# anuragranj/cc

Measured on AMD Instinct MI355X. Metric: train images/sec (832x256, 5-frame sample, 6-scale CC step), higher is better.
Workload: dtype f32; 1 GPU; full CC: DispResNet6+PoseNetB6+MaskNet6+Back2Future, all losses; per_gpu_batch=4, global_batch=4, height=256, width=832, scales=6, frames=5, parallelism=dp1, hipgraph=True, trained_nets=all, rccl_ranks=1, dead_occlusion_decoders_elided=False, net_streams=2, pipeline=per_network, grad_chunks=False, deterministic=True

## Files before the change

### cc_amd/csrc/conv_wgrad.hip

```cpp
#include <stdio.h>
#include <stddef.h>
#include <string.h>
#include "cc_common.h"
#include "conv_internal.h"
#include "cc_tools.h"
#include "../../include/ccengine.h"

namespace {

typedef float f32x16 __attribute__((ext_vector_type(16)));

using ccint::BK;
using ccint::BN;
using ccint::MAXGRP;
using ccint::pick_bm;

struct WG {
    const float* a;
    const float* x;
    float* out;
    const float* ga[MAXGRP]; const float* gxp[MAXGRP]; float* gout[MAXGRP];
    int nsplit;
    int B, M, AH, AW; long a_bs;
    int Cin, IH, IW; long x_bs;
    int Rt, St, dy0, dx0, dstep, si;
    long o_sm, o_sc; int o_ri, o_sj;
    int direct, accum;
    int pix_per_split;
};

template <int BM>
__device__ __forceinline__ void wgrad_body(const WG& g, const int bx_, const int by_, const int bz_) {
    const int grp = bz_ / g.nsplit, zsplit = bz_ - grp * g.nsplit;
    const float* __restrict__ a_ = g.ga[grp];
    const float* __restrict__ x_ = g.gxp[grp];
    float* __restrict__ out_ = g.gout[grp];
    constexpr int WM = (BM >= 64) ? BM / 2 : 32;
    constexpr int WN = (BM >= 64) ? 64 : 32;
    constexpr int TM = WM / 32, TN = WN / 32;
    constexpr int AP = BM + 4, BP = BN + 4;
    constexpr int AQ = BM / 16;
    __shared__ float As[2][BK * AP];
    __shared__ float Bs[2][BK * BP];

    const int tid = threadIdx.x, lane = tid & 63;
    const int wid = __builtin_amdgcn_readfirstlane(tid >> 6);
    const int wm = (BM >= 64) ? (wid >> 1) : 0;
    const int wn = (BM >= 64) ? (wid & 1) : wid;
    const int m0 = by_ * BM;
    const int n0 = bx_ * BN;
    const int RS = g.Rt * g.St;
    const int Ntot = g.Cin * RS;
    const int HWa = g.AH * g.AW;
    const long Ptot = (long)g.B * HWa;
    const long pbeg = (long)zsplit * g.pix_per_split;
    long pend = pbeg + g.pix_per_split;
    if (pend > Ptot) pend = Ptot;
    const int x_cs = g.IH * g.IW;

    const int pp = tid & 15, rgp = tid >> 4;
    int xoff[8], tdy[8], tdx[8];
#pragma unroll
    for (int q = 0; q < 8; q++) {
        const int jn = n0 + rgp + 16 * q;
        if (jn < Ntot) {
            const int c = jn / RS, rem = jn - c * RS;
            const int i = rem / g.St, j = rem - i * g.St;
            tdy[q] = g.dy0 + i * g.dstep;
            tdx[q] = g.dx0 + j * g.dstep;
            xoff[q] = c * x_cs + tdy[q] * g.IW + tdx[q];
        } else {
            tdy[q] = -(1 << 28);
            tdx[q] = 0;
            xoff[q] = 0;
        }
    }
    float ra[AQ], rb[8];
    unsigned okA = 0, okB = 0;
    auto load_chunk = [&](long pbase) {
        okA = 0;
        okB = 0;
        const long p = pbase + pp;
        const bool pv = p < pend;
        const long ps = pv ? p : 0;
        const int n = (int)(ps / HWa);
        const int t = (int)(ps - (long)n * HWa);
        const int ty = t / g.AW, tx = t - ty * g.AW;
        const long abase = (long)n * g.a_bs + ty * g.AW + tx;
#pragma unroll
        for (int q = 0; q < AQ; q++) {
            const int m = m0 + rgp + 16 * q;
            const bool ok = pv && (m < g.M);
            ra[q] = a_[ok ? abase + (long)m * HWa : 0];
            okA |= (ok ? 1u : 0u) << q;
        }
        const int iy0 = g.si * ty, ix0 = g.si * tx;
        const long xb = (long)n * g.x_bs + (long)iy0 * g.IW + ix0;
#pragma unroll
        for (int q = 0; q < 8; q++) {
            const int iy = iy0 + tdy[q], ix = ix0 + tdx[q];
            const bool ok = pv && ((unsigned)iy < (unsigned)g.IH) && ((unsigned)ix < (unsigned)g.IW);
            rb[q] = x_[ok ? xb + xoff[q] : 0];
            okB |= (ok ? 1u : 0u) << q;
        }
    };
    auto store_chunk = [&](int buf) {
#pragma unroll
        for (int q = 0; q < AQ; q++) As[buf][pp * AP + rgp + 16 * q] = ((okA >> q) & 1u) ? ra[q] : 0.f;
#pragma unroll
        for (int q = 0; q < 8; q++) Bs[buf][pp * BP + rgp + 16 * q] = ((okB >> q) & 1u) ? rb[q] : 0.f;
    };

    f32x16 acc[TM][TN];
#pragma unroll
    for (int a = 0; a < TM; a++)
#pragma unroll
        for (int b = 0; b < TN; b++)
#pragma unroll
            for (int r = 0; r < 16; r++) acc[a][b][r] = 0.f;

    const int l31 = lane & 31, lk = lane >> 5;
    const long nchunks = (pend > pbeg) ? (pend - pbeg + BK - 1) / BK : 0;
    if (nchunks > 0) {
        load_chunk(pbeg);
        store_chunk(0);
    }
    __syncthreads();
    for (long ch = 0; ch < nchunks; ch++) {
        const int buf = (int)(ch & 1);
        if (ch + 1 < nchunks) load_chunk(pbeg + (ch + 1) * BK);
        {
            float af[BK / 2][TM], bf[BK / 2][TN];
#pragma unroll
            for (int ks = 0; ks < BK / 2; ks++) {
#pragma unroll
                for (int a = 0; a < TM; a++) af[ks][a] = As[buf][(2 * ks + lk) * AP + wm * WM + a * 32 + l31];
#pragma unroll
                for (int b = 0; b < TN; b++) bf[ks][b] = Bs[buf][(2 * ks + lk) * BP + wn * WN + b * 32 + l31];
            }
#pragma unroll
            for (int ks = 0; ks < BK / 2; ks++)
#pragma unroll
                for (int a = 0; a < TM; a++)
#pragma unroll
                    for (int b = 0; b < TN; b++)
                        acc[a][b] = __builtin_amdgcn_mfma_f32_32x32x2f32(af[ks][a], bf[ks][b], acc[a][b], 0, 0, 0);
        }
        if (ch + 1 < nchunks) store_chunk(buf ^ 1);
        __syncthreads();
    }
#pragma unroll
    for (int b = 0; b < TN; b++) {
        const int jn = n0 + wn * WN + b * 32 + l31;
        if (jn >= Ntot) continue;
        long obase;
        if (g.direct) {
            const int c = jn / RS, rem = jn - c * RS;
            const int i = rem / g.St, j = rem - i * g.St;
            obase = (long)c * g.o_sc + i * g.o_ri + j * g.o_sj;
        } else {
            obase = (long)zsplit * g.M * Ntot + jn;
        }
#pragma unroll
        for (int a = 0; a < TM; a++)
#pragma unroll
            for (int r = 0; r < 16; r++) {
                const int m = m0 + wm * WM + a * 32 + (r & 3) + 8 * (r >> 2) + 4 * lk;
                if (m < g.M) {
                    float* o = out_ + obase + (g.direct ? (long)m * g.o_sm : (long)m * Ntot);
                    *o = (g.direct && g.accum) ? (*o + acc[a][b][r]) : acc[a][b][r];
                }
            }
    }
}

template <int BM>
__global__ __launch_bounds__(256) void k_wgrad(WG g) {
    if constexpr (CC_XCD_MASK & 4) {
        const int gx = (int)gridDim.x, gy = (int)gridDim.y;
        const int b = cc_xcd_order((int)blockIdx.x + gx * ((int)blockIdx.y + gy * (int)blockIdx.z), gx * gy * (int)gridDim.z);
        const int r = b / gx;
        wgrad_body<BM>(g, b - r * gx, r % gy, r / gy);
    } else {
        wgrad_body<BM>(g, (int)blockIdx.x, (int)blockIdx.y, (int)blockIdx.z);
    }
}

constexpr int MAXWCLS = 12;
struct WGM { WG c[MAXWCLS]; int n; int bx_end[MAXWCLS]; int gx[MAXWCLS], gy[MAXWCLS]; };
template <int BM>
__global__ __launch_bounds__(256) void k_wgrad_multi(WGM a) {
    int k = 0, first = 0, end = a.bx_end[0];
#pragma unroll
    for (int q = 0; q < MAXWCLS - 1; q++)
        if (q + 1 < a.n && (int)blockIdx.x >= a.bx_end[q]) { k = q + 1; first = a.bx_end[q]; end = a.bx_end[q + 1]; }
#if defined(__HIP_DEVICE_COMPILE__) && !defined(CC_HIPEMU)
    const WG& g = *(reinterpret_cast<const WG*>((const char*)__builtin_amdgcn_kernarg_segment_ptr() + offsetof(WGM, c)) + k);
#else
    const WG& g = a.c[k];
#endif
    const int b = (CC_XCD_MASK & 4) ? cc_xcd_order((int)blockIdx.x - first, end - first) : (int)blockIdx.x - first;
    const int gx = a.gx[k], gy = a.gy[k];
    const int bx = b % gx, r = b / gx;
    wgrad_body<BM>(g, bx, r % gy, r / gy);
}

constexpr int W3_PC = 41;

struct W3 {
    const float* a; const float* x; const float* zeros; float* ws;
    const float* ga[MAXGRP]; const float* gxp[MAXGRP]; float* gws[MAXGRP];
    int B, M, AH, AW; long a_bs;
    int Cin; long x_bs;
    int tiles_x, tiles_y, ntiles, tiles_per_split, nsplit, Cpad, dbg;
};

template <int MT, int CT>
__global__ __launch_bounds__(256, 2) void k_wgrad3x3(W3 g) {
    const float* __restrict__ a_ = g.ga[blockIdx.y];
    const float* __restrict__ x_ = g.gxp[blockIdx.y];
    float* __restrict__ ws_ = g.gws[blockIdx.y];
    constexpr int BM = 32 * MT, BC = 32 * CT;
    constexpr int A_SLOTS = BM * 16;
    constexpr int P_SLOTS = ((BC * W3_PC + 63) / 64) * 64;
    HIP_DYNAMIC_SHARED(float, smem)
    float4* As = reinterpret_cast<float4*>(smem);
    float4* Ps = reinterpret_cast<float4*>(smem) + A_SLOTS;

    const int tid = threadIdx.x, lane = tid & 63;
    const int wid = __builtin_amdgcn_readfirstlane(tid >> 6);
    const int l31 = lane & 31, lk = lane >> 5;
    const int ctiles = g.Cpad / BC;
    const int ctile = blockIdx.x % ctiles, mtile = blockIdx.x / ctiles;
    const int m0 = mtile * BM, c0 = ctile * BC;
    const int HW = g.AH * g.AW;
    const int pt_beg = blockIdx.z * g.tiles_per_split;
    int pt_end = pt_beg + g.tiles_per_split;
    if (pt_end > g.ntiles) pt_end = g.ntiles;

    int g_row[3], g_mt[3], g_ct[3];
    f32x16 acc[3][3];
#pragma unroll
    for (int k = 0; k < 3; k++) {
        const int gi = wid + 4 * k;
        g_row[k] = gi % 3;
        const int tl = gi / 3;
        g_mt[k] = tl % MT;
        g_ct[k] = tl / MT;
#pragma unroll
        for (int j = 0; j < 3; j++)
#pragma unroll
            for (int r = 0; r < 16; r++) acc[k][j][r] = 0.f;
    }

    auto load_tile = [&](int pt) {
        const int tile_x = pt % g.tiles_x;
        const int r2 = pt / g.tiles_x;
        const int tile_y = r2 % g.tiles_y;
        const int n = r2 / g.tiles_y;
        const int ty0 = tile_y * 2, tx0 = tile_x * 32;
        for (int s0 = wid * 64; s0 < A_SLOTS; s0 += 256) {
            const int sl = s0 + lane;
            const int mm = sl >> 4, sc = sl & 15;
            const int pc = sc ^ (mm & 15);
            const int ty = ty0 + (pc >> 3), tx = tx0 + 4 * (pc & 7);
            const int m = m0 + mm;
            const bool ok = (m < g.M) && (ty < g.AH) && (tx < g.AW);
            const float* src = ok ? a_ + (long)n * g.a_bs + (long)m * HW + (long)ty * g.AW + tx : g.zeros;
            __builtin_amdgcn_global_load_lds(CC_GLOBAL_PTR(src), CC_LDS_PTR(As + s0), 16, 0, 0);
        }
        for (int s0 = wid * 64; s0 < P_SLOTS; s0 += 256) {
            const int sl = s0 + lane;
            const int cc = sl / W3_PC, r = sl - cc * W3_PC;
            const int py = r / 10, ch = r - py * 10;
            const int iy = ty0 - 1 + py, ix = tx0 - 4 + 4 * ch;
            const int c = c0 + cc;
            const bool ok = (cc < BC) && (r < 40) && (c < g.Cin) && ((unsigned)iy < (unsigned)g.AH) && ((unsigned)ix < (unsigned)g.AW);
            const float* src = ok ? x_ + (long)n * g.x_bs + (long)c * HW + (long)iy * g.AW + ix : g.zeros;
            __builtin_amdgcn_global_load_lds(CC_GLOBAL_PTR(src), CC_LDS_PTR(Ps + s0), 16, 0, 0);
        }
    };

    for (int pt = pt_beg; pt < pt_end; pt++) {
        if (pt > pt_beg) __syncthreads();
        if (!(g.dbg & 1) || pt == pt_beg) load_tile(pt);
        CC_WAIT_VMCNT0();
        __syncthreads();
        if (g.dbg & 2) continue;
#pragma unroll
        for (int row = 0; row < 2; row++) {
#pragma unroll 2
            for (int pq = 0; pq < 4; pq++) {
#pragma unroll
                for (int k = 0; k < 3; k++) {
                    const int mrow = g_mt[k] * 32 + l31;
                    float4 av = As[mrow * 16 + ((row * 8 + pq + 4 * lk) ^ (mrow & 15))];
                    const float4* Pr = Ps + (g_ct[k] * 32 + l31) * W3_PC + (row + g_row[k]) * 10 + 4 * lk + pq;
                    float4 w0 = Pr[0], w1 = Pr[1], w2 = Pr[2];
                    CC_KEEP4(av); CC_KEEP4(w0); CC_KEEP4(w1); CC_KEEP4(w2);
                    const float a[4] = {av.x, av.y, av.z, av.w};
                    const float w[12] = {w0.x, w0.y, w0.z, w0.w, w1.x, w1.y, w1.z, w1.w, w2.x, w2.y, w2.z, w2.w};
#pragma unroll
                    for (int e = 0; e < 4; e++)
#pragma unroll
                        for (int j = 0; j < 3; j++)
                            acc[k][j] = __builtin_amdgcn_mfma_f32_32x32x2f32(a[e], w[3 + j + e], acc[k][j], 0, 0, 0);
                }
            }
        }
    }
#pragma unroll
    for (int k = 0; k < 3; k++) {
#pragma unroll
        for (int j = 0; j < 3; j++) {
            float* o = ws_ + (((long)blockIdx.z * 9 + (g_row[k] * 3 + j)) * g.M) * g.Cpad + c0 + g_ct[k] * 32 + l31;
#pragma unroll
            for (int r = 0; r < 16; r++) {
                const int m = m0 + g_mt[k] * 32 + (r & 3) + 8 * (r >> 2) + 4 * lk;
                if (m < g.M) o[(long)m * g.Cpad] = acc[k][j][r];
            }
        }
    }
}

__global__ void k_zero64(float* p) { p[threadIdx.x] = 0.f; }

struct WgGeom { int B, M, AH, AW, Cin, IH, IW, R, S, si, pad; };

struct W3Plan { bool ok; int mt, nbuf, tiles_x, tiles_y, ntiles, nsplit, tps, Cp32; size_t smem, ws_floats; };

inline W3Plan plan_w3(int B, int M, int AH, int AW, int Cin, int R, int S, int si, int pad, int IH, int IW, int G = 1) {
    W3Plan p = {};
    p.ok = (R == 3 && S == 3 && si == 1 && pad == 1 && IH == AH && IW == AW && (AW % 4) == 0 && AW >= 16 && Cin >= 32 &&
            M >= cctools::env_int("CC_W3_MINM", 64) &&
            !cctools::env_flag("CC_NO_WGRAD3X3"));
    if (!p.ok) return p;
    p.mt = (M > 64) ? 4 : ((M > 32 && Cin > 32) ? 2 : ((Cin > 64) ? 1 : 2));
    p.nbuf = 1;
    const int BM = 32 * p.mt, BC = 32 * (4 / p.mt);
    p.Cp32 = ((Cin + BC - 1) / BC) * BC;
    p.tiles_x = (AW + 31) / 32;
    p.tiles_y = (AH + 1) / 2;
    p.ntiles = B * p.tiles_x * p.tiles_y;
    const long base = (long)((M + BM - 1) / BM) * (p.Cp32 / BC) * (G > 1 ? G : 1);
    long nsplit = (cctools::env_int("CC_W3_SPLIT", 512) + base - 1) / base;
    const long mt_ = cctools::env_int("CC_W3_MINTILES", 3);
    const long cap = (p.ntiles + mt_ - 1) / mt_;
    if (nsplit > cap) nsplit = cap;
    if (nsplit > p.ntiles) nsplit = p.ntiles;
    if (nsplit < 1) nsplit = 1;
    p.tps = (int)((p.ntiles + nsplit - 1) / nsplit);
    p.nsplit = (p.ntiles + p.tps - 1) / p.tps;
    p.smem = (size_t)(BM * 16 + ((BC * W3_PC + 63) / 64) * 64) * 16;
    p.ws_floats = 64 + (size_t)p.nsplit * 9 * M * p.Cp32;
    return p;
}

struct WinoPadPlan { bool ok; int Wp; ccint::WinoWgradPlan wp; size_t pad_floats; };
inline WinoPadPlan wino_pad_plan(int B, int M, int AH, int AW, int Cin, int G) {
    WinoPadPlan p = {};
    if ((AW % 4) == 0 || AH < 2 || cctools::env_flag("CC_NO_WINO_WGRAD_PAD")) return p;
    if (M < cctools::env_int("CC_WWP_MINM", 96) || Cin < cctools::env_int("CC_WWP_MINC", 96)) return p;
    p.Wp = (AW + 3) & ~3;
    p.wp = ccint::wino_wgrad_plan(B, M, AH, p.Wp, Cin, G, cctools::env_int("CC_WWP_MINQ", 64));
    p.ok = p.wp.ok != 0;
    p.pad_floats = ((size_t)B * (Cin + M) * AH * p.Wp + 3) & ~(size_t)3;
    return p;
}

inline long generic_nsplit(long tiles, long P, bool parked) {
    const long target = parked ? cctools::env_int("CC_WGRAD_PARK_TARGET", 256) : cctools::env_int("CC_WGRAD_SPLIT_TARGET", 512);
    long nsplit = (target + tiles - 1) / tiles;
    const long mr = parked ? cctools::env_int("CC_WGRAD_PARK_MINRANGE", 64) : cctools::env_int("CC_WGRAD_MINRANGE", 32);
    const long maxsplit = (P + mr - 1) / mr;
    if (nsplit > maxsplit) nsplit = maxsplit;
    return nsplit < 1 ? 1 : nsplit;
}

enum WgPath { WG_WINO, WG_WINO_PAD, WG_HEAD, WG_THIN, WG_W3, WG_GENERIC };
struct WgCand {
    WgPath path;
    size_t ws_floats;
    char name[64];
    ccint::WinoWgradPlan wino; int Wp;
    ccint::HeadWgradPlan head;
    W3Plan w3;
};
constexpr int WG_MAXCAND = 5;

static int wgrad_candidates(const WgGeom& g, int G, bool sizing, WgCand* out) {
    int n = 0;
    auto add = [&](WgPath path, size_t ws_floats) -> WgCand& {
        out[n] = WgCand{};
        out[n].path = path;
        out[n].ws_floats = ws_floats;
        return out[n++];
    };
    const int pad = sizing ? 1 : g.pad, IH = sizing ? g.AH : g.IH, IW = sizing ? g.AW : g.IW;
    if (g.R == 3 && g.S == 3 && g.si == 1 && pad == 1 && IH == g.AH && IW == g.AW) {
        const ccint::WinoWgradPlan wp = ccint::wino_wgrad_plan(g.B, g.M, g.AH, g.AW, g.Cin, G);
        if (wp.ok) {
            WgCand& c = add(WG_WINO, wp.ws_floats);
            c.wino = wp;
            snprintf(c.name, sizeof c.name, "k_wino_wgrad");
        }
        const WinoPadPlan pp = wino_pad_plan(g.B, g.M, g.AH, g.AW, g.Cin, G);
        if (pp.ok) {
            WgCand& c = add(WG_WINO_PAD, pp.wp.ws_floats + pp.pad_floats);
            c.wino = pp.wp;
            c.Wp = pp.Wp;
            snprintf(c.name, sizeof c.name, "k_wino_wgrad");
        }
        const ccint::HeadWgradPlan hp = g.M <= 2 ? ccint::head_wgrad_plan(g.B, g.M, g.AH, g.AW, g.Cin) : ccint::HeadWgradPlan{};
        if (hp.ok) {
            WgCand& c = add(WG_HEAD, hp.ws_floats);
            c.head = hp;
            snprintf(c.name, sizeof c.name, "k_wgrad_thinm<%d>", g.M);
        }
    }
    {
        char nm[64] = "";
        if (!sizing) ccint::wgrad_thin_name(g.B, g.M, g.AH, g.AW, g.Cin, g.IH, g.IW, g.R, g.S, g.si, g.pad, nm, sizeof nm);
        const size_t wf = ccint::wgrad_thin_ws_floats(g.B, g.M, g.AH, g.AW, g.Cin, g.R, g.S, g.si);
        if (wf && (sizing || nm[0])) memcpy(add(WG_THIN, wf).name, nm, sizeof nm);
    }
    const W3Plan q = plan_w3(g.B, g.M, g.AH, g.AW, g.Cin, g.R, g.S, g.si, pad, IH, IW, G);
    if (q.ok) {
        WgCand& c = add(WG_W3, q.ws_floats);
        c.w3 = q;
        snprintf(c.name, sizeof c.name, "k_wgrad3x3<%d, %d>", q.mt, 4 / q.mt);
    } else {
        const long Ntot = (long)g.Cin * g.R * g.S;
        const int bm = pick_bm(g.M);
        const long nsplit = generic_nsplit(((Ntot + BN - 1) / BN) * ((g.M + bm - 1) / bm), (long)g.B * g.AH * g.AW, false);
        WgCand& c = add(WG_GENERIC, nsplit <= 1 ? 4 : (size_t)nsplit * g.M * Ntot);
        snprintf(c.name, sizeof c.name, "k_wgrad<%d>", bm);
    }
    return n;
}

struct WgradParked { WG g; int bm; dim3 grid; double gflop; };
struct WgradCollector { WgradParked* p; int cap, n; ccint::WinoWgradParked* wino; };

static void launch_wgrad_parked(const WgradCollector& c, hipStream_t s) {
    for (int bm = 128; bm >= 32; bm /= 2) {
        int i = 0;
        while (i < c.n) {
            WGM m = {};
            long blk = 0;
            double gf = 0;
            for (; i < c.n && m.n < MAXWCLS; i++) {
                if (c.p[i].bm != bm) continue;
                const dim3& gr = c.p[i].grid;
                const long nb = (long)gr.x * gr.y * gr.z;
                if (m.n && blk + nb >= (1l << 31)) break;
                m.c[m.n] = c.p[i].g;
                m.gx[m.n] = (int)gr.x; m.gy[m.n] = (int)gr.y;
                blk += nb;
                m.bx_end[m.n] = (int)blk;
                gf += c.p[i].gflop;
                m.n++;
            }
            if (!m.n) break;
            char nm[64];
            snprintf(nm, sizeof nm, "k_wgrad_multi<%d>%s", bm, "");
            cctiming::Scope tsc(nm, gf, s);
            if (bm == 128) hipLaunchKernelGGL(HIP_KERNEL_NAME(k_wgrad_multi<128>), dim3((unsigned)blk), dim3(256), 0, s, m);
            else if (bm == 64) hipLaunchKernelGGL(HIP_KERNEL_NAME(k_wgrad_multi<64>), dim3((unsigned)blk), dim3(256), 0, s, m);
            else hipLaunchKernelGGL(HIP_KERNEL_NAME(k_wgrad_multi<32>), dim3((unsigned)blk), dim3(256), 0, s, m);
        }
    }
}

struct WgCall {
    int G; const long *a, *x, *gw;
    float* ws; size_t stride_f;
    WgGeom g; long a_bs, x_bs, o_sm, o_sc; int accumulate;
    hipStream_t s; ccint::RedSink* sink; const float* zeros64; WgradCollector* park;
    float* area(int k) const { return ws + k * stride_f; }
};
constexpr int WG_DECLINED = 1;

static int emit_slab_reduce(const WgCall& c, float* const* slabs, int nsplit, int Cp) {
    long rd[MAXGRP][ccint::RD_LONGS];
    for (int k = 0; k < c.G; k++) {
        const long d[ccint::RD_LONGS] = {1, (long)slabs[k], (long)c.gw[k], nsplit, c.accumulate, c.o_sm, c.o_sc, 9, c.g.M, c.g.Cin, Cp};
        memcpy(rd[k], d, sizeof d);
    }
    return ccint::wgrad_reduce_emit(c.sink, &rd[0][0], c.G, c.s);
}

static int emit_tile_reduce(const WgCall& c, long nsplit) {
    const WgGeom& g = c.g;
    long rd[MAXGRP][ccint::RD_LONGS];
    for (int k = 0; k < c.G; k++) {
        const long d[ccint::RD_LONGS] = {0, (long)c.area(k), (long)c.gw[k], nsplit, c.accumulate, c.o_sm, c.o_sc, g.M,
                                         (long)g.Cin * g.R * g.S, g.R * g.S, g.S, g.S, 1};
        memcpy(rd[k], d, sizeof d);
    }
    return ccint::wgrad_reduce_emit(c.sink, &rd[0][0], c.G, c.s);
}

static int run_wino(const WgCall& c, const WgCand& cd) {
    const WgGeom& g = c.g;
    const bool padded = cd.path == WG_WINO_PAD;
    const int W = padded ? cd.Wp : g.AW;
    ccint::WinoWgradParked* wpark = c.park ? c.park->wino : nullptr;
    const bool parks = wpark && wpark->n + c.G <= ccint::WINO_WGRAD_PARK_CAP;
    const ccint::WinoWgradPlan wp = parks ? ccint::wino_wgrad_plan_parked(cd.wino, g.M) : cd.wino;
    const size_t slabs = (cd.wino.ws_floats + 3) & ~(size_t)3;
    const float *ap[MAXGRP], *xp[MAXGRP];
    float* wsp[MAXGRP];
    ccint::PadJob jobs[2 * MAXGRP];
    for (int k = 0; k < c.G; k++) {
        ap[k] = (const float*)c.a[k]; xp[k] = (const float*)c.x[k]; wsp[k] = c.area(k) + 64;
        if (padded) {
            float* xpad = c.area(k) + slabs;
            float* apad = xpad + (size_t)g.B * g.Cin * g.AH * W;
            jobs[2 * k] = ccint::PadJob{xp[k], xpad, c.x_bs, g.Cin * g.AH};
            jobs[2 * k + 1] = ccint::PadJob{ap[k], apad, c.a_bs, g.M * g.AH};
            xp[k] = xpad; ap[k] = apad;
        }
    }
    char nm[128];
    int nl = snprintf(nm, sizeof nm, "%s", cd.name);
    if (cctools::env_flag("CC_TIMING_DETAIL")) {
        nl += snprintf(nm + nl, sizeof nm - nl, " G%d B%d M%d C%d %dx%d", c.G, g.B, g.M, g.Cin, g.AH, g.AW);
        if (padded) nl += snprintf(nm + nl, sizeof nm - nl, "(pad %d)", W);
        snprintf(nm + nl, sizeof nm - nl, " k%d wg%d", wp.nsplit, wp.nmb * wp.ncb * c.G * wp.nsplit);
    }
    bool ok;
    {
        cctiming::Scope tsc(nm, 2e-9 * 16.0 * c.G * g.B * ((g.AH + 1) / 2) * ((W + 1) / 2) * (double)g.M * g.Cin, c.s, !parks);
        if (padded) ccint::pad_rows_launch(jobs, 2 * c.G, g.B, g.AW, W, c.s);
        ok = ccint::wino_wgrad_launch(wp, ap, xp, wsp, c.G, g.B, g.M, g.AH, W, padded ? (long)g.M * g.AH * W : c.a_bs, g.Cin,
                                      padded ? (long)g.Cin * g.AH * W : c.x_bs, c.s, wpark);
    }
    return ok ? emit_slab_reduce(c, wsp, wp.nsplit, wp.Cp) : WG_DECLINED;
}

static int run_head(const WgCall& c, const WgCand& cd) {
    const WgGeom& g = c.g;
    const ccint::HeadWgradPlan& hp = cd.head;
    char nm[128];
    const int nl = snprintf(nm, sizeof nm, "%s", cd.name);
    if (cctools::env_flag("CC_TIMING_DETAIL"))
        snprintf(nm + nl, sizeof nm - nl, " G%d B%d M%d C%d %dx%d r3 s1 k%d", c.G, g.B, g.M, g.Cin, g.AH, g.AW, hp.nblk);
    bool ok = true;
    {
        cctiming::Scope tsc(nm, 2e-9 * c.G * g.B * g.AH * g.AW * (double)g.M * g.Cin * 9, c.s);
        for (int k = 0; k < c.G && ok; k++)
            ok = ccint::head_wgrad_launch(hp, (const float*)c.a[k], (const float*)c.x[k], c.area(k), g.B, g.M, g.AH, g.AW, c.a_bs, g.Cin,
                                          c.x_bs, c.s);
    }
    if (!ok) return WG_DECLINED;
    if (cctools::env_flag("CC_HEAD_TRACE"))
        fprintf(stderr, "head wgrad: G%d B%d M%d C%d %dx%d R%d nblk %d\n", c.G, g.B, g.M, g.Cin, g.AH, g.AW, hp.R, hp.nblk);
    return emit_tile_reduce(c, hp.nblk);
}

static int run_thin(const WgCall& c, const WgCand& cd) {
    const WgGeom& g = c.g;
    char nm[128];
    const int nl = snprintf(nm, sizeof nm, "%s", cd.name);
    if (cctools::env_flag("CC_TIMING_DETAIL"))
        snprintf(nm + nl, sizeof nm - nl, " G%d B%d M%d C%d %dx%d r%d s%d", c.G, g.B, g.M, g.Cin, g.AH, g.AW, g.R, g.si);
    cctiming::Scope tsc(nm, 2e-9 * c.G * g.B * g.AH * g.AW * (double)g.M * g.Cin * g.R * g.S, c.s, !ccint::wgrad_thin_parking());
    bool thin = true;
    for (int k = 0; k < c.G && thin; k++)
        thin = ccint::wgrad_thin_launch((const float*)c.a[k], (const float*)c.x[k], (float*)c.gw[k], c.area(k), g.B, g.M, g.AH, g.AW,
                                        c.a_bs, g.Cin, g.IH, g.IW, c.x_bs, g.R, g.S, g.si, g.pad, c.o_sm, c.o_sc, c.accumulate, c.s,
                                        c.sink);
    return thin ? CC_OK : WG_DECLINED;
}

static int run_w3(const WgCall& c, const WgCand& cd) {
    const WgGeom& g = c.g;
    const W3Plan& q = cd.w3;
    W3 w = {};
    w.zeros = c.zeros64 ? c.zeros64 : c.ws;
    for (int k = 0; k < c.G; k++) { w.ga[k] = (const float*)c.a[k]; w.gxp[k] = (const float*)c.x[k]; w.gws[k] = c.area(k) + 64; }
    w.B = g.B; w.M = g.M; w.AH = g.AH; w.AW = g.AW; w.a_bs = c.a_bs; w.Cin = g.Cin; w.x_bs = c.x_bs;
    w.tiles_x = q.tiles_x; w.tiles_y = q.tiles_y; w.ntiles = q.ntiles; w.tiles_per_split = q.tps; w.nsplit = q.nsplit;
    w.Cpad = q.Cp32;
    if (!c.zeros64) hipLaunchKernelGGL(k_zero64, dim3(1), dim3(64), 0, c.s, c.ws);
    const int BM = 32 * q.mt, BC = 32 * (4 / q.mt);
    dim3 grid((unsigned)(((g.M + BM - 1) / BM) * (q.Cp32 / BC)), (unsigned)c.G, (unsigned)q.nsplit);
    w.dbg = cctools::env_int("CC_W3_DBG", 0);
    {
        char nm[128];
        const int nl = snprintf(nm, sizeof nm, "%s", cd.name);
        if (cctools::env_flag("CC_TIMING_DETAIL"))
            snprintf(nm + nl, sizeof nm - nl, " G%d B%d M%d C%d %dx%d k%d wg%d", c.G, g.B, g.M, g.Cin, g.AH, g.AW, q.nsplit,
                     (int)(grid.x * grid.y * grid.z));
        cctiming::Scope tsc(nm, 2e-9 * c.G * g.B * g.AH * g.AW * (double)g.M * g.Cin * 9, c.s);
        if (q.mt == 4) hipLaunchKernelGGL(HIP_KERNEL_NAME(k_wgrad3x3<4, 1>), grid, dim3(256), q.smem, c.s, w);
        else if (q.mt == 2) hipLaunchKernelGGL(HIP_KERNEL_NAME(k_wgrad3x3<2, 2>), grid, dim3(256), q.smem, c.s, w);
        else hipLaunchKernelGGL(HIP_KERNEL_NAME(k_wgrad3x3<1, 4>), grid, dim3(256), q.smem, c.s, w);
    }
    return emit_slab_reduce(c, w.gws, q.nsplit, q.Cp32);
}

static int run_generic(const WgCall& c, const WgCand& cd) {
    const WgGeom& g = c.g;
    const long Ntot = (long)g.Cin * g.R * g.S;
    const long P = (long)g.B * g.AH * g.AW;
    const int bm = pick_bm(g.M);
    const bool parked = c.park && c.park->n < c.park->cap;
    long nsplit = generic_nsplit(((Ntot + BN - 1) / BN) * ((g.M + bm - 1) / bm) * c.G, P, parked);
    long pps = (P + nsplit - 1) / nsplit;
    pps = ((pps + BK - 1) / BK) * BK;
    nsplit = (P + pps - 1) / pps;
    WG w = {};
    w.B = g.B; w.M = g.M; w.AH = g.AH; w.AW = g.AW; w.a_bs = c.a_bs;
    w.Cin = g.Cin; w.IH = g.IH; w.IW = g.IW; w.x_bs = c.x_bs;
    w.Rt = g.R; w.St = g.S; w.dy0 = -g.pad; w.dx0 = -g.pad; w.dstep = 1; w.si = g.si;
    w.o_sm = c.o_sm; w.o_sc = c.o_sc; w.o_ri = g.S; w.o_sj = 1;
    w.direct = (nsplit == 1);
    w.accum = c.accumulate;
    w.nsplit = (int)nsplit;
    for (int k = 0; k < c.G; k++) {
        w.ga[k] = (const float*)c.a[k]; w.gxp[k] = (const float*)c.x[k];
        w.gout[k] = w.direct ? (float*)c.gw[k] : c.area(k);
    }
    w.pix_per_split = (int)pps;
    dim3 grid((unsigned)((Ntot + BN - 1) / BN), (unsigned)((g.M + bm - 1) / bm), (unsigned)(nsplit * c.G));
    const double gflop = 2e-9 * c.G * g.B * g.AH * g.AW * (double)g.M * g.Cin * g.R * g.S;
    if (parked) {
        c.park->p[c.park->n++] = WgradParked{w, bm, grid, gflop};
    } else {
        char nm[128];
        const int nl = snprintf(nm, sizeof nm, "%s", cd.name);
        if (cctools::env_flag("CC_TIMING_DETAIL"))
            snprintf(nm + nl, sizeof nm - nl, " G%d B%d M%d C%d %dx%d r%d s%d k%ld wg%d", c.G, g.B, g.M, g.Cin, g.AH, g.AW, g.R, g.si,
                     (long)nsplit, (int)(grid.x * grid.y * grid.z));
        cctiming::Scope tsc(nm, gflop, c.s);
        if (bm == 128) hipLaunchKernelGGL(HIP_KERNEL_NAME(k_wgrad<128>), grid, dim3(256), 0, c.s, w);
        else if (bm == 64) hipLaunchKernelGGL(HIP_KERNEL_NAME(k_wgrad<64>), grid, dim3(256), 0, c.s, w);
        else hipLaunchKernelGGL(HIP_KERNEL_NAME(k_wgrad<32>), grid, dim3(256), 0, c.s, w);
    }
    return w.direct ? CC_OK : emit_tile_reduce(c, nsplit);
}

}

extern "C" {

size_t cc_conv2d_wgrad_ws_bytes(int B, int M, int AH, int AW, int Cin, int R, int S, int si) {
    const WgGeom g = {B, M, AH, AW, Cin, 0, 0, R, S, si, 0};
    WgCand c[WG_MAXCAND];
    size_t floats = 0;
    for (int G = 1; G <= MAXGRP; G++) {
        const int n = wgrad_candidates(g, G, true, c);
        for (int i = 0; i < n; i++)
            if (c[i].ws_floats > floats) floats = c[i].ws_floats;
    }
    return (floats * sizeof(float) + 15) & ~(size_t)15;
}

static int wgrad_group_impl(int G, const long* a, const long* x, const long* gw, float* ws, int B, int M, int AH, int AW, long a_bs,
                            int Cin, int IH, int IW, long x_bs, int R, int S, int si, int pad, long o_sm, long o_sc, int accumulate,
                            void* stream, ccint::RedSink* sink, const float* zeros64 = nullptr, WgradCollector* park = nullptr) {
    if (G <= 0 || G > MAXGRP || B <= 0 || M <= 0 || Cin <= 0) return CC_ERR_ARG;
    const WgCall c = {G, a, x, gw, ws, cc_conv2d_wgrad_ws_bytes(B, M, AH, AW, Cin, R, S, si) / sizeof(float),
                      WgGeom{B, M, AH, AW, Cin, IH, IW, R, S, si, pad}, a_bs, x_bs, o_sm, o_sc, accumulate,
                      (hipStream_t)stream, sink, zeros64, park};
    WgCand cand[WG_MAXCAND];
    const int n = wgrad_candidates(c.g, G, false, cand);
    for (int i = 0; i < n; i++) {
        const WgCand& cd = cand[i];
        const int r = cd.path == WG_WINO || cd.path == WG_WINO_PAD ? run_wino(c, cd)
                      : cd.path == WG_HEAD ? run_head(c, cd)
                      : cd.path == WG_THIN ? run_thin(c, cd)
                      : cd.path == WG_W3   ? run_w3(c, cd)
                                           : run_generic(c, cd);
        if (r == WG_DECLINED) continue;
        if (r != CC_OK) return CC_ERR_ARG;
        CC_CHECK_LAUNCH();
        return CC_OK;
    }
    return CC_ERR_ARG;
}

int cc_conv2d_wgrad_group(int G, const long* a, const long* x, const long* gw, float* ws, int B, int M, int AH, int AW, long a_bs,
                          int Cin, int IH, int IW, long x_bs, int R, int S, int si, int pad, long o_sm, long o_sc, int accumulate,
                          void* stream) {
    return wgrad_group_impl(G, a, x, gw, ws, B, M, AH, AW, a_bs, Cin, IH, IW, x_bs, R, S, si, pad, o_sm, o_sc, accumulate, stream,
                            nullptr);
}

int cc_conv2d_wgrad_group_defer(int G, const long* a, const long* x, const long* gw, float* ws, int B, int M, int AH, int AW,
                                long a_bs, int Cin, int IH, int IW, long x_bs, int R, int S, int si, int pad, long o_sm, long o_sc,
                                int accumulate, const float* zeros64_or_null, long* red_host, int red_cap, int* nred_host,
                                void* stream) {
    if (!red_host || !nred_host || red_cap < G) return CC_ERR_ARG;
    ccint::RedSink sink = {red_host, red_cap, 0};
    const int r = wgrad_group_impl(G, a, x, gw, ws, B, M, AH, AW, a_bs, Cin, IH, IW, x_bs, R, S, si, pad, o_sm, o_sc, accumulate,
                                   stream, &sink, zeros64_or_null);
    *nred_host = sink.n;
    return r;
}

int cc_conv2d_wgrad_list(int n, const long* desc_host, const float* zeros64_or_null, long* red_host, int red_cap, int* nred_host,
                         void* stream) {
    if (n <= 0 || !desc_host || !red_host || !nred_host) return CC_ERR_ARG;
    hipStream_t s = (hipStream_t)stream;
    constexpr int CAP = 64;
    static thread_local WgradParked parked[CAP];
    static thread_local ccint::WinoWgradParked wino_parked;
    wino_parked.n = 0;
    WgradCollector col = {parked, CAP, 0, cctools::env_flag("CC_NO_WINO_WGRAD_LIST") ? nullptr : &wino_parked};
    ccint::RedSink sink = {red_host, red_cap, 0};
    struct ThinPark {
        hipStream_t s; bool was;
        explicit ThinPark(hipStream_t st) : s(st), was(ccint::wgrad_thin_park(true)) {}
        ~ThinPark() {
            const double gf = ccint::wgrad_thin_parked_gflop();
            if (gf > 0) {
                cctiming::Scope tsc("k_wgrad_thin_multi", gf, s);
                ccint::wgrad_thin_flush(s);
            }
            ccint::wgrad_thin_park(was);
        }
    } thin_park(s);
    for (int i = 0; i < n; i++) {
        const long* d = desc_host + 32l * i;
        const int G = (int)d[0];
        auto bail = [&](int code) {
            launch_wgrad_parked(col, s);
            if (wino_parked.n > 0) ccint::wino_wgrad_launch_parked(&wino_parked, s);
            *nred_host = sink.n;
            return code;
        };
        if (G <= 0 || G > MAXGRP || sink.n + G > red_cap) return bail(CC_ERR_ARG);
        const int before = col.n;
        const int r = wgrad_group_impl(G, d + 1, d + 5, d + 9, (float*)d[13], (int)d[14], (int)d[15], (int)d[16], (int)d[17], d[18],
                                       (int)d[19], (int)d[20], (int)d[21], d[22], (int)d[23], (int)d[24], (int)d[25], (int)d[26], d[27],
                                       d[28], (int)d[29], stream, &sink, zeros64_or_null, &col);
        if (r != CC_OK) return bail(r);
        if (col.n > before && col.p[before].g.direct) {
            bool dup = false;
            for (int j = 0; j < before && !dup; j++)
                if (col.p[j].g.direct)
                    for (int u = 0; u < MAXGRP && !dup; u++)
                        for (int v = 0; v < MAXGRP; v++)
                            if (col.p[j].g.gout[u] && col.p[j].g.gout[u] == col.p[before].g.gout[v]) { dup = true; break; }
            if (dup) {
                const WgradParked keep = col.p[before];
                col.n = before;
                launch_wgrad_parked(col, s);
                col.p[0] = keep;
                col.n = 1;
            }
        }
    }
    launch_wgrad_parked(col, s);
    if (wino_parked.n > 0) {
        double gf = 0;
        for (int i = 0; i < wino_parked.n; i++) gf += wino_parked.d[i].gflop;
        cctiming::Scope tsc("k_wino_wgrad_multi", gf, s);
        ccint::wino_wgrad_launch_parked(&wino_parked, s);
    }
    *nred_host = sink.n;
    CC_CHECK_LAUNCH();
    return CC_OK;
}

int cc_conv2d_wgrad(const float* a, const float* x, float* gw, float* ws, int B, int M, int AH, int AW, long a_bs, int Cin,
                    int IH, int IW, long x_bs, int R, int S, int si, int pad, long o_sm, long o_sc, int accumulate, void* stream) {
    const long ap = (long)a, xp = (long)x, gp = (long)gw;
    return cc_conv2d_wgrad_group(1, &ap, &xp, &gp, ws, B, M, AH, AW, a_bs, Cin, IH, IW, x_bs, R, S, si, pad, o_sm, o_sc, accumulate,
                                 stream);
}

int cc_conv2d_wgrad_kernel(int B, int M, int AH, int AW, int Cin, int IH, int IW, int R, int S, int si, int pad,
                           void* name_out_host, int cap) {
    WgCand c[WG_MAXCAND];
    wgrad_candidates(WgGeom{B, M, AH, AW, Cin, IH, IW, R, S, si, pad}, 1, false, c);
    snprintf((char*)name_out_host, cap, "%s", c[0].name);
    return CC_OK;
}

}
```

Measured before the change: 250.5 images/s.

## Add vectorized wgrad loads, incremental pixel indexing and register double-buffering

The generic weight-gradient kernel gains form variants. When the activation gradient is 16-byte aligned, its loads become float4 reads along pixels. For 1x1 stride-1 unpadded convolutions the input loads also become float4. Per-chunk pixel division is replaced with incremental carry updates, and for BM=128 tiles a two-stage register pipeline with sched barriers and occupancy 2 launch bounds is added. It aims to cut global load instruction count and index arithmetic, at the cost of higher register pressure and more code paths.

```diff
diff --git a/cc_amd/csrc/conv_wgrad.hip b/cc_amd/csrc/conv_wgrad.hip
--- a/cc_amd/csrc/conv_wgrad.hip
+++ b/cc_amd/csrc/conv_wgrad.hip
@@ -27,21 +27,321 @@
     long o_sm, o_sc; int o_ri, o_sj;
     int direct, accum;
     int pix_per_split;
+    int form;
 };
 
+constexpr int WF_AWIDE = 1;
+constexpr int WF_XPIX = 4;
+constexpr int WF_LEGACY = 8;
+
+#if defined(__HIP_DEVICE_COMPILE__) && !defined(CC_HIPEMU)
+#define WG_PIN(v) asm volatile("" : "+v"(v))
+#else
+#define WG_PIN(v) ((void)0)
+#endif
+
+typedef float f32x4 __attribute__((ext_vector_type(4)));
+
+struct WgYes { static constexpr bool value = true; };
+struct WgNo { static constexpr bool value = false; };
+
+template <int BM> struct WgTile {
+    static constexpr int WM = (BM >= 64) ? BM / 2 : 32;
+    static constexpr int WN = (BM >= 64) ? 64 : 32;
+    static constexpr int TM = WM / 32, TN = WN / 32;
+    static constexpr int AP = BM + 4, BP = BN + 4;
+    static constexpr int AQ = BM / 16;
+};
+
+template <int BM, int ABL>
+__device__ __forceinline__ void wgrad_chunk(const float* As, const float* Bs, f32x16 (&acc)[WgTile<BM>::TM][WgTile<BM>::TN], int wm, int wn,
+                                            int l31, int lk) {
+    using T = WgTile<BM>;
+    float af[BK / 2][T::TM], bf[BK / 2][T::TN];
+#pragma unroll
+    for (int ks = 0; ks < BK / 2; ks++) {
+#pragma unroll
+        for (int a = 0; a < T::TM; a++) af[ks][a] = As[(2 * ks + lk) * T::AP + wm * T::WM + a * 32 + l31];
+#pragma unroll
+        for (int b = 0; b < T::TN; b++) bf[ks][b] = Bs[(2 * ks + lk) * T::BP + wn * T::WN + b * 32 + l31];
+    }
+#pragma unroll
+    for (int ks = 0; ks < BK / 2; ks++)
+#pragma unroll
+        for (int a = 0; a < T::TM; a++)
+#pragma unroll
+            for (int b = 0; b < T::TN; b++) {
+                if constexpr (ABL & 2) acc[a][b][0] = fmaf(af[ks][a], bf[ks][b], acc[a][b][0]);
+                else acc[a][b] = __builtin_amdgcn_mfma_f32_32x32x2f32(af[ks][a], bf[ks][b], acc[a][b], 0, 0, 0);
+            }
+}
+
 template <int BM>
-__device__ __forceinline__ void wgrad_body(const WG& g, const int bx_, const int by_, const int bz_) {
+__device__ __forceinline__ void wgrad_write(const WG& g, float* __restrict__ out_, const f32x16 (&acc)[WgTile<BM>::TM][WgTile<BM>::TN],
+                                            int m0, int n0, int zsplit, int wm, int wn, int l31, int lk) {
+    using T = WgTile<BM>;
+    const int RS = g.Rt * g.St;
+    const int Ntot = g.Cin * RS;
+#pragma unroll
+    for (int b = 0; b < T::TN; b++) {
+        const int jn = n0 + wn * T::WN + b * 32 + l31;
+        if (jn >= Ntot) continue;
+        long obase;
+        if (g.direct) {
+            const int c = jn / RS, rem = jn - c * RS;
+            const int i = rem / g.St, j = rem - i * g.St;
+            obase = (long)c * g.o_sc + i * g.o_ri + j * g.o_sj;
+        } else {
+            obase = (long)zsplit * g.M * Ntot + jn;
+        }
+#pragma unroll
+        for (int a = 0; a < T::TM; a++)
+#pragma unroll
+            for (int r = 0; r < 16; r++) {
+                const int m = m0 + wm * T::WM + a * 32 + (r & 3) + 8 * (r >> 2) + 4 * lk;
+                if (m < g.M) {
+                    float* o = out_ + obase + (g.direct ? (long)m * g.o_sm : (long)m * Ntot);
+                    *o = (g.direct && g.accum) ? (*o + acc[a][b][r]) : acc[a][b][r];
+                }
+            }
+    }
+}
+
+template <int BM, int AF, int XF>
+__device__ __forceinline__ void wgrad_body(const WG& g, float* As, float* Bs, const int bx_, const int by_, const int bz_) {
+    using T = WgTile<BM>;
+    constexpr int AP = T::AP, BP = T::BP, AQ = T::AQ;
     const int grp = bz_ / g.nsplit, zsplit = bz_ - grp * g.nsplit;
     const float* __restrict__ a_ = g.ga[grp];
     const float* __restrict__ x_ = g.gxp[grp];
     float* __restrict__ out_ = g.gout[grp];
-    constexpr int WM = (BM >= 64) ? BM / 2 : 32;
-    constexpr int WN = (BM >= 64) ? 64 : 32;
-    constexpr int TM = WM / 32, TN = WN / 32;
-    constexpr int AP = BM + 4, BP = BN + 4;
-    constexpr int AQ = BM / 16;
-    __shared__ float As[2][BK * AP];
-    __shared__ float Bs[2][BK * BP];
+
+    const int tid = threadIdx.x, lane = tid & 63;
+    const int wid = __builtin_amdgcn_readfirstlane(tid >> 6);
+    const int wm = (BM >= 64) ? (wid >> 1) : 0;
+    const int wn = (BM >= 64) ? (wid & 1) : wid;
+    const int m0 = by_ * BM;
+    const int n0 = bx_ * BN;
+    const int RS = g.Rt * g.St;
+    const int Ntot = g.Cin * RS;
+    const int HWa = g.AH * g.AW;
+    const long Ptot = (long)g.B * HWa;
+    const long pbeg = (long)zsplit * g.pix_per_split;
+    long pend = pbeg + g.pix_per_split;
+    if (pend > Ptot) pend = Ptot;
+    const int plen = pend > pbeg ? (int)(pend - pbeg) : 0;
+    const int x_cs = g.IH * g.IW;
+
+    const int pp = tid & 15, rgp = tid >> 4;
+    const int pg = tid & 3, r4 = tid >> 2;
+    constexpr int QA = (BM >= 64) ? BM / 64 : 1;
+    constexpr int NA = AF ? 4 * QA : AQ;
+    constexpr int NB = 8;
+    struct Stage { float a[NA]; float b[NB]; unsigned okA, okB; };
+
+    int xoff[8], tdy[8], tdx[8];
+    if constexpr (XF == 0) {
+#pragma unroll
+        for (int q = 0; q < 8; q++) {
+            const int jn = n0 + rgp + 16 * q;
+            if (jn < Ntot) {
+                const int c = jn / RS, rem = jn - c * RS;
+                const int i = rem / g.St, j = rem - i * g.St;
+                tdy[q] = g.dy0 + i * g.dstep;
+                tdx[q] = g.dx0 + j * g.dstep;
+                xoff[q] = c * x_cs + tdy[q] * g.IW + tdx[q];
+            } else {
+                tdy[q] = -(1 << 28);
+                tdx[q] = 0;
+                xoff[q] = 0;
+            }
+        }
+    }
+
+    const int q16 = BK / HWa, r16 = BK - q16 * HWa;
+    const int qW = BK / g.AW, rW = BK - qW * g.AW;
+    const int dty = qW - q16 * g.AH;
+    int en, ety, etx, wn_, wt;
+    {
+        const long p = pbeg + pp;
+        en = (int)(p / HWa);
+        const int t = (int)(p - (long)en * HWa);
+        ety = t / g.AW;
+        etx = t - ety * g.AW;
+        const long pw = pbeg + 4 * pg;
+        wn_ = (int)(pw / HWa);
+        wt = (int)(pw - (long)wn_ * HWa);
+    }
+    int done = 0;
+
+    auto load_chunk = [&](Stage& s) {
+        s.okA = 0;
+        s.okB = 0;
+        const bool pv = done + pp < plen;
+        const bool pvw = done + 4 * pg < plen;
+        if constexpr (AF) {
+            const long abase = (long)wn_ * g.a_bs + wt;
+#pragma unroll
+            for (int q = 0; q < QA; q++) {
+                const int m = m0 + r4 + 64 * q;
+                const bool ok = pvw && (m < g.M) && (BM >= 64 || r4 < BM);
+                const f32x4 v = *reinterpret_cast<const f32x4*>(a_ + (ok ? abase + (long)m * HWa : 0));
+                s.a[4 * q] = v.x; s.a[4 * q + 1] = v.y; s.a[4 * q + 2] = v.z; s.a[4 * q + 3] = v.w;
+                s.okA |= (ok ? 1u : 0u) << q;
+            }
+        } else {
+            const long abase = (long)en * g.a_bs + ety * g.AW + etx;
+#pragma unroll
+            for (int q = 0; q < AQ; q++) {
+                const int m = m0 + rgp + 16 * q;
+                const bool ok = pv && (m < g.M);
+                s.a[q] = a_[ok ? abase + (long)m * HWa : 0];
+                s.okA |= (ok ? 1u : 0u) << q;
+            }
+        }
+        if constexpr (XF == 0) {
+            const int iy0 = g.si * ety, ix0 = g.si * etx;
+            const long xb = (long)en * g.x_bs + (long)iy0 * g.IW + ix0;
+#pragma unroll
+            for (int q = 0; q < 8; q++) {
+                const int iy = iy0 + tdy[q], ix = ix0 + tdx[q];
+                const bool ok = pv && ((unsigned)iy < (unsigned)g.IH) && ((unsigned)ix < (unsigned)g.IW);
+                s.b[q] = x_[ok ? xb + xoff[q] : 0];
+                s.okB |= (ok ? 1u : 0u) << q;
+            }
+        } else {
+            const long xb = (long)wn_ * g.x_bs + wt;
+#pragma unroll
+            for (int q = 0; q < 2; q++) {
+                const int jn = n0 + r4 + 64 * q;
+                const bool ok = pvw && (jn < Ntot);
+                const f32x4 v = *reinterpret_cast<const f32x4*>(x_ + (ok ? xb + (long)jn * HWa : 0));
+                s.b[4 * q] = v.x; s.b[4 * q + 1] = v.y; s.b[4 * q + 2] = v.z; s.b[4 * q + 3] = v.w;
+                s.okB |= (ok ? 1u : 0u) << q;
+            }
+        }
+        done += BK;
+        etx += rW;
+        const int cy = etx >= g.AW ? 1 : 0;
+        etx -= cy ? g.AW : 0;
+        ety += dty + cy;
+        const int cn = ety >= g.AH ? 1 : 0;
+        ety -= cn ? g.AH : 0;
+        en += q16 + cn;
+        wt += r16;
+        const int cw = wt >= HWa ? 1 : 0;
+        wt -= cw ? HWa : 0;
+        wn_ += q16 + cw;
+    };
+    auto store_chunk = [&](Stage& s, int buf) {
+        float* A = As + buf * (BK * AP);
+        float* Bt = Bs + buf * (BK * BP);
+        if constexpr (AF) {
+            if (BM >= 64 || r4 < BM) {
+#pragma unroll
+                for (int q = 0; q < QA; q++)
+#pragma unroll
+                    for (int e = 0; e < 4; e++) A[(4 * pg + e) * AP + r4 + 64 * q] = ((s.okA >> q) & 1u) ? s.a[4 * q + e] : 0.f;
+            }
+        } else {
+#pragma unroll
+            for (int q = 0; q < AQ; q++) A[pp * AP + rgp + 16 * q] = ((s.okA >> q) & 1u) ? s.a[q] : 0.f;
+        }
+        if constexpr (XF == 0) {
+#pragma unroll
+            for (int q = 0; q < 8; q++) Bt[pp * BP + rgp + 16 * q] = ((s.okB >> q) & 1u) ? s.b[q] : 0.f;
+        } else {
+#pragma unroll
+            for (int q = 0; q < 2; q++)
+#pragma unroll
+                for (int e = 0; e < 4; e++) Bt[(4 * pg + e) * BP + r4 + 64 * q] = ((s.okB >> q) & 1u) ? s.b[4 * q + e] : 0.f;
+        }
+    };
+
+    f32x16 acc[T::TM][T::TN];
+#pragma unroll
+    for (int a = 0; a < T::TM; a++)
+#pragma unroll
+        for (int b = 0; b < T::TN; b++)
+#pragma unroll
+            for (int r = 0; r < 16; r++) acc[a][b][r] = 0.f;
+
+    const int l31 = lane & 31, lk = lane >> 5;
+    const int nchunks = (plen + BK - 1) / BK;
+    Stage s0, s1;
+    auto step = [&](auto ldc, auto stc, int ch, Stage& ld, Stage& st) {
+        const int buf = ch & 1;
+        if constexpr (decltype(ldc)::value) {
+            load_chunk(ld);
+            __builtin_amdgcn_sched_barrier(0);
+        }
+        wgrad_chunk<BM, 0>(As + buf * (BK * AP), Bs + buf * (BK * BP), acc, wm, wn, l31, lk);
+        if constexpr (decltype(stc)::value) {
+            __builtin_amdgcn_sched_barrier(0);
+#pragma unroll
+            for (int q = 0; q < NA; q++) WG_PIN(st.a[q]);
+#pragma unroll
+            for (int q = 0; q < NB; q++) WG_PIN(st.b[q]);
+            store_chunk(st, buf ^ 1);
+        }
+        __syncthreads();
+    };
+    constexpr WgYes yes = {};
+    constexpr WgNo no = {};
+    if constexpr (BM < 128) {
+        if (nchunks > 0) {
+            load_chunk(s0);
+            store_chunk(s0, 0);
+        }
+        __syncthreads();
+        for (int ch = 0; ch < nchunks; ch++) {
+            const int buf = ch & 1;
+            if (ch + 1 < nchunks) load_chunk(s0);
+            wgrad_chunk<BM, 0>(As + buf * (BK * AP), Bs + buf * (BK * BP), acc, wm, wn, l31, lk);
+            if (ch + 1 < nchunks) store_chunk(s0, buf ^ 1);
+            __syncthreads();
+        }
+    } else if (nchunks > 0) {
+        load_chunk(s0);
+        store_chunk(s0, 0);
+        int ch = 0;
+        if (nchunks & 1) {
+            if (nchunks > 1) {
+                load_chunk(s0);
+                __syncthreads();
+                step(yes, yes, 0, s1, s0);
+                ch = 1;
+            } else {
+                __syncthreads();
+                ch = -1;
+            }
+        } else {
+            load_chunk(s1);
+            __syncthreads();
+        }
+        if (ch >= 0) {
+            for (; ch + 2 < nchunks; ch += 2) {
+                step(yes, yes, ch, s0, s1);
+                step(yes, yes, ch + 1, s1, s0);
+            }
+            step(no, yes, ch, s0, s1);
+        }
+        step(no, no, nchunks - 1, s1, s0);
+    }
+    wgrad_write<BM>(g, out_, acc, m0, n0, zsplit, wm, wn, l31, lk);
+}
+
+#ifdef CC_TOOLS
+template <int BM, int ABL>
+__device__ __forceinline__ void wgrad_body_legacy(const WG& g, float* As_, float* Bs_, const int bx_, const int by_, const int bz_) {
+    using T = WgTile<BM>;
+    constexpr int AP = T::AP, BP = T::BP, AQ = T::AQ;
+    const int grp = bz_ / g.nsplit, zsplit = bz_ - grp * g.nsplit;
+    const float* __restrict__ a_ = g.ga[grp];
+    const float* __restrict__ x_ = g.gxp[grp];
+    float* __restrict__ out_ = g.gout[grp];
+    float (*As)[BK * AP] = reinterpret_cast<float (*)[BK * AP]>(As_);
+    float (*Bs)[BK * BP] = reinterpret_cast<float (*)[BK * BP]>(Bs_);
 
     const int tid = threadIdx.x, lane = tid & 63;
     const int wid = __builtin_amdgcn_readfirstlane(tid >> 6);
@@ -111,11 +411,11 @@
         for (int q = 0; q < 8; q++) Bs[buf][pp * BP + rgp + 16 * q] = ((okB >> q) & 1u) ? rb[q] : 0.f;
     };
 
-    f32x16 acc[TM][TN];
-#pragma unroll
-    for (int a = 0; a < TM; a++)
-#pragma unroll
-        for (int b = 0; b < TN; b++)
+    f32x16 acc[T::TM][T::TN];
+#pragma unroll
+    for (int a = 0; a < T::TM; a++)
+#pragma unroll
+        for (int b = 0; b < T::TN; b++)
 #pragma unroll
             for (int r = 0; r < 16; r++) acc[a][b][r] = 0.f;
 
@@ -128,68 +428,57 @@
     __syncthreads();
     for (long ch = 0; ch < nchunks; ch++) {
         const int buf = (int)(ch & 1);
-        if (ch + 1 < nchunks) load_chunk(pbeg + (ch + 1) * BK);
-        {
-            float af[BK / 2][TM], bf[BK / 2][TN];
-#pragma unroll
-            for (int ks = 0; ks < BK / 2; ks++) {
-#pragma unroll
-                for (int a = 0; a < TM; a++) af[ks][a] = As[buf][(2 * ks + lk) * AP + wm * WM + a * 32 + l31];
-#pragma unroll
-                for (int b = 0; b < TN; b++) bf[ks][b] = Bs[buf][(2 * ks + lk) * BP + wn * WN + b * 32 + l31];
-            }
-#pragma unroll
-            for (int ks = 0; ks < BK / 2; ks++)
-#pragma unroll
-                for (int a = 0; a < TM; a++)
-#pragma unroll
-                    for (int b = 0; b < TN; b++)
-                        acc[a][b] = __builtin_amdgcn_mfma_f32_32x32x2f32(af[ks][a], bf[ks][b], acc[a][b], 0, 0, 0);
-        }
+        if (!(ABL & 1) && ch + 1 < nchunks) load_chunk(pbeg + (ch + 1) * BK);
+        wgrad_chunk<BM, ABL>(As[buf], Bs[buf], acc, wm, wn, l31, lk);
         if (ch + 1 < nchunks) store_chunk(buf ^ 1);
         __syncthreads();
     }
-#pragma unroll
-    for (int b = 0; b < TN; b++) {
-        const int jn = n0 + wn * WN + b * 32 + l31;
-        if (jn >= Ntot) continue;
-        long obase;
-        if (g.direct) {
-            const int c = jn / RS, rem = jn - c * RS;
-            const int i = rem / g.St, j = rem - i * g.St;
-            obase = (long)c * g.o_sc + i * g.o_ri + j * g.o_sj;
-        } else {
-            obase = (long)zsplit * g.M * Ntot + jn;
-        }
-#pragma unroll
-        for (int a = 0; a < TM; a++)
-#pragma unroll
-            for (int r = 0; r < 16; r++) {
-                const int m = m0 + wm * WM + a * 32 + (r & 3) + 8 * (r >> 2) + 4 * lk;
-                if (m < g.M) {
-                    float* o = out_ + obase + (g.direct ? (long)m * g.o_sm : (long)m * Ntot);
-                    *o = (g.direct && g.accum) ? (*o + acc[a][b][r]) : acc[a][b][r];
-                }
-            }
-    }
-}
+    wgrad_write<BM>(g, out_, acc, m0, n0, zsplit, wm, wn, l31, lk);
+}
+#endif
 
 template <int BM>
-__global__ __launch_bounds__(256) void k_wgrad(WG g) {
+__device__ __forceinline__ void wgrad_tile(const WG& g, const int bx, const int by, const int bz) {
+    using T = WgTile<BM>;
+    __shared__ __attribute__((aligned(16))) float As[2 * BK * T::AP];
+    __shared__ __attribute__((aligned(16))) float Bs[2 * BK * T::BP];
+    switch (g.form) {
+    case 0: wgrad_body<BM, 0, 0>(g, As, Bs, bx, by, bz); break;
+    case WF_AWIDE: wgrad_body<BM, 1, 0>(g, As, Bs, bx, by, bz); break;
+    case WF_XPIX: wgrad_body<BM, 0, 2>(g, As, Bs, bx, by, bz); break;
+    case WF_AWIDE | WF_XPIX: wgrad_body<BM, 1, 2>(g, As, Bs, bx, by, bz); break;
+#ifdef CC_TOOLS
+    default: wgrad_body_legacy<BM, 0>(g, As, Bs, bx, by, bz); break;
+#endif
+    }
+}
+
+template <int BM>
+__global__ __launch_bounds__(256, BM == 128 ? 2 : 1) void k_wgrad(WG g) {
     if constexpr (CC_XCD_MASK & 4) {
         const int gx = (int)gridDim.x, gy = (int)gridDim.y;
         const int b = cc_xcd_order((int)blockIdx.x + gx * ((int)blockIdx.y + gy * (int)blockIdx.z), gx * gy * (int)gridDim.z);
         const int r = b / gx;
-        wgrad_body<BM>(g, b - r * gx, r % gy, r / gy);
+        wgrad_tile<BM>(g, b - r * gx, r % gy, r / gy);
     } else {
-        wgrad_body<BM>(g, (int)blockIdx.x, (int)blockIdx.y, (int)blockIdx.z);
-    }
-}
+        wgrad_tile<BM>(g, (int)blockIdx.x, (int)blockIdx.y, (int)blockIdx.z);
+    }
+}
+
+#ifdef CC_TOOLS
+template <int ABL>
+__global__ __launch_bounds__(256) void k_wgrad_abl(WG g) {
+    using T = WgTile<128>;
+    __shared__ __attribute__((aligned(16))) float As[2 * BK * T::AP];
+    __shared__ __attribute__((aligned(16))) float Bs[2 * BK * T::BP];
+    wgrad_body_legacy<128, ABL>(g, As, Bs, (int)blockIdx.x, (int)blockIdx.y, (int)blockIdx.z);
+}
+#endif
 
 constexpr int MAXWCLS = 12;
 struct WGM { WG c[MAXWCLS]; int n; int bx_end[MAXWCLS]; int gx[MAXWCLS], gy[MAXWCLS]; };
 template <int BM>
-__global__ __launch_bounds__(256) void k_wgrad_multi(WGM a) {
+__global__ __launch_bounds__(256, BM == 128 ? 2 : 1) void k_wgrad_multi(WGM a) {
     int k = 0, first = 0, end = a.bx_end[0];
 #pragma unroll
     for (int q = 0; q < MAXWCLS - 1; q++)
@@ -202,7 +491,7 @@
     const int b = (CC_XCD_MASK & 4) ? cc_xcd_order((int)blockIdx.x - first, end - first) : (int)blockIdx.x - first;
     const int gx = a.gx[k], gy = a.gy[k];
     const int bx = b % gx, r = b / gx;
-    wgrad_body<BM>(g, bx, r % gy, r / gy);
+    wgrad_tile<BM>(g, bx, r % gy, r / gy);
 }
 
 constexpr int W3_PC = 41;
@@ -449,12 +738,14 @@
             WGM m = {};
             long blk = 0;
             double gf = 0;
+            int ngrp[MAXWCLS] = {};
             for (; i < c.n && m.n < MAXWCLS; i++) {
                 if (c.p[i].bm != bm) continue;
                 const dim3& gr = c.p[i].grid;
                 const long nb = (long)gr.x * gr.y * gr.z;
                 if (m.n && blk + nb >= (1l << 31)) break;
                 m.c[m.n] = c.p[i].g;
+                ngrp[m.n] = (int)gr.z / c.p[i].g.nsplit;
                 m.gx[m.n] = (int)gr.x; m.gy[m.n] = (int)gr.y;
                 blk += nb;
                 m.bx_end[m.n] = (int)blk;
@@ -462,8 +753,24 @@
                 m.n++;
             }
             if (!m.n) break;
-            char nm[64];
-            snprintf(nm, sizeof nm, "k_wgrad_multi<%d>%s", bm, "");
+            char nm[768];
+            int nl = snprintf(nm, sizeof nm, "k_wgrad_multi<%d>", bm);
+            if (cctools::env_flag("CC_TIMING_DETAIL")) {
+                for (int k = 0; k < m.n && nl < (int)sizeof nm - 64; k++) {
+                    const WG& g = m.c[k];
+                    int same = 0, first = 1;
+                    for (int j = 0; j < m.n; j++) {
+                        const WG& h = m.c[j];
+                        const bool eq = h.B == g.B && h.M == g.M && h.Cin == g.Cin && h.AH == g.AH && h.AW == g.AW && h.Rt == g.Rt &&
+                                        h.St == g.St && h.si == g.si && h.nsplit == g.nsplit;
+                        if (eq) { same += ngrp[j]; if (j < k) first = 0; }
+                    }
+                    if (!first) continue;
+                    nl += snprintf(nm + nl, sizeof nm - nl, " %dx[B%d M%d C%d %dx%d r%d s%d k%d]", same, g.B, g.M, g.Cin, g.AH, g.AW, g.Rt,
+                                   g.si, g.nsplit);
+                }
+                snprintf(nm + nl, sizeof nm - nl, " wg%ld", blk);
+            }
             cctiming::Scope tsc(nm, gf, s);
             if (bm == 128) hipLaunchKernelGGL(HIP_KERNEL_NAME(k_wgrad_multi<128>), dim3((unsigned)blk), dim3(256), 0, s, m);
             else if (bm == 64) hipLaunchKernelGGL(HIP_KERNEL_NAME(k_wgrad_multi<64>), dim3((unsigned)blk), dim3(256), 0, s, m);
@@ -601,6 +908,22 @@
     return emit_slab_reduce(c, w.gws, q.nsplit, q.Cp32);
 }
 
+static int generic_form(const WgCall& c) {
+    const WgGeom& g = c.g;
+    if (cctools::env_flag("CC_WGRAD_SCALAR")) return WF_LEGACY;
+    auto aligned16 = [&](const long* p) {
+        for (int k = 0; k < c.G; k++)
+            if (p[k] & 15) return false;
+        return true;
+    };
+    const long HWa = (long)g.AH * g.AW;
+    int f = 0;
+    if (HWa % 4 == 0 && c.a_bs % 4 == 0 && aligned16(c.a)) f |= WF_AWIDE;
+    if (g.R == 1 && g.S == 1 && g.si == 1 && g.pad == 0 && g.IH == g.AH && g.IW == g.AW && HWa % 4 == 0 && c.x_bs % 4 == 0 && aligned16(c.x))
+        f |= WF_XPIX;
+    return f;
+}
+
 static int run_generic(const WgCall& c, const WgCand& cd) {
     const WgGeom& g = c.g;
     const long Ntot = (long)g.Cin * g.R * g.S;
@@ -624,6 +947,10 @@
         w.gout[k] = w.direct ? (float*)c.gw[k] : c.area(k);
     }
     w.pix_per_split = (int)pps;
+    w.form = generic_form(c);
+    if (cctools::env_flag("CC_WGRAD_TRACE"))
+        fprintf(stderr, "wgrad generic: %dx[B%d M%d C%d %dx%d r%d s%d] bm %d nsplit %ld pps %ld form %d%s\n", c.G, g.B, g.M, g.Cin, g.AH, g.AW,
+                g.R, g.si, bm, nsplit, pps, w.form, parked ? " parked" : "");
     dim3 grid((unsigned)((Ntot + BN - 1) / BN), (unsigned)((g.M + bm - 1) / bm), (unsigned)(nsplit * c.G));
     const double gflop = 2e-9 * c.G * g.B * g.AH * g.AW * (double)g.M * g.Cin * g.R * g.S;
     if (parked) {
@@ -635,6 +962,13 @@
             snprintf(nm + nl, sizeof nm - nl, " G%d B%d M%d C%d %dx%d r%d s%d k%ld wg%d", c.G, g.B, g.M, g.Cin, g.AH, g.AW, g.R, g.si,
                      (long)nsplit, (int)(grid.x * grid.y * grid.z));
         cctiming::Scope tsc(nm, gflop, c.s);
+#ifdef CC_TOOLS
+        const int abl = (w.form & WF_LEGACY) ? cctools::env_int("CC_WGRAD_ABL", 0) : 0;
+        if (bm == 128 && abl == 1) hipLaunchKernelGGL(HIP_KERNEL_NAME(k_wgrad_abl<1>), grid, dim3(256), 0, c.s, w);
+        else if (bm == 128 && abl == 2) hipLaunchKernelGGL(HIP_KERNEL_NAME(k_wgrad_abl<2>), grid, dim3(256), 0, c.s, w);
+        else if (bm == 128 && abl == 3) hipLaunchKernelGGL(HIP_KERNEL_NAME(k_wgrad_abl<3>), grid, dim3(256), 0, c.s, w);
+        else
+#endif
         if (bm == 128) hipLaunchKernelGGL(HIP_KERNEL_NAME(k_wgrad<128>), grid, dim3(256), 0, c.s, w);
         else if (bm == 64) hipLaunchKernelGGL(HIP_KERNEL_NAME(k_wgrad<64>), grid, dim3(256), 0, c.s, w);
         else hipLaunchKernelGGL(HIP_KERNEL_NAME(k_wgrad<32>), grid, dim3(256), 0, c.s, w);
```

Result: no change. 251.3 images/s, median of 6 (+0.3%).
